# weiyithu/PV-RAFT

Hardware: NVIDIA H100
Metric: raft_sample_iters_per_sec (higher is better)
Workload: dtype f32

## Files before the change

pvraft_b200/csrc/tc_linear.cu:

```cuda
#include <cuda.h>
#include <stdlib.h>

#include "fixed_point.cuh"
#include "wgmma.cuh"

namespace pvraft {

constexpr int kTcThreads = 544;
constexpr int kTcEpiThreads = 256, kTcProducerWarp = 16;
constexpr int kTcM = 128, kTcKB = 32;
constexpr int kTcABytes = kTcM * kTcKB * 4;
constexpr int kTcMaxStages = 6;

#ifdef PVRAFT_TC_TIMELINE
__device__ unsigned long long g_tc_clock[64];
__device__ __forceinline__ unsigned long long gtimer() { unsigned long long t; asm volatile("mov.u64 %0, %%globaltimer;" : "=l"(t)); return t; }
#define TC_MARK(cond, slot) do { if (clk && (cond)) g_tc_clock[(slot)] = gtimer(); } while (0)
#else
#define TC_MARK(cond, slot) do { } while (0)
#endif

enum TcEpilogue { TC_EPI_PLAIN = 0, TC_EPI_GRU_ZR = 1, TC_EPI_GRU_Q = 2, TC_EPI_FLOW = 3 };

struct TcParams {
    const double* in_stats;
    const float* in_gamma;
    const float* in_beta;
    double in_count;
    int in_act;
    float in_slope;
    int minmax;
    int epi;
    const float* bias;
    const float* bias2;
    int out_act;
    const float* residual;
    float* out;
    float* out2;
    const float* h;
    const float* z;
    double* out_stats;
    int M, N, K, cout, pts_per_sample;
    const float* src[3];
    const float* src_min;
    int seg_kb[3];
    int stages;
    int w_resident;
    int settled;
    int dbg;
    int gn_kb;
    int out_ld;
    const float* tail;
// ... 259 lines not shown
                    const float4 aq = __ldg(reinterpret_cast<const float4*>(p.residual + (size_t)row * 64 + c + q * 4));
                    bq.x += aq.x; bq.y += aq.y; bq.z += aq.z; bq.w += aq.w;
                }
                o[q * 4 + 0] = tgru_blend(zv.x, hv.x, __uint_as_float(vq[q * 4 + 0]) + bq.x);
                o[q * 4 + 1] = tgru_blend(zv.y, hv.y, __uint_as_float(vq[q * 4 + 1]) + bq.y);
                o[q * 4 + 2] = tgru_blend(zv.z, hv.z, __uint_as_float(vq[q * 4 + 2]) + bq.z);
                o[q * 4 + 3] = tgru_blend(zv.w, hv.w, __uint_as_float(vq[q * 4 + 3]) + bq.w);
            }
            stage_store16(stg, lane, o, p.out + (size_t)(row0 + quad * 32) * 64 + c, 64);
        }
    }
}


struct TcCursor {
    int ti = 0, kb = 0, s = 0;
    unsigned phase = 0;
    __device__ __forceinline__ void next(int num_kb, int S) {
        if (++kb == num_kb) { kb = 0; ++ti; }
        if (++s == S) { s = 0; phase ^= 1u; }
    }
};

template <int N>
__device__ __forceinline__ void tc_mma_kblock(float (&acc)[64], unsigned long long a_hi, unsigned long long a_lo, unsigned long long b_hi,
                                              unsigned long long b_lo, int kb) {
#pragma unroll
    for (int k = 0; k < kTcKB / 8; ++k) {
        wgmma_tf32<N>(acc, wgmma_desc_k(a_hi, k), wgmma_desc_k(b_hi, k), (kb | k) != 0);
        wgmma_tf32<N>(acc, wgmma_desc_k(a_lo, k), wgmma_desc_k(b_hi, k), 1);
        wgmma_tf32<N>(acc, wgmma_desc_k(a_hi, k), wgmma_desc_k(b_lo, k), 1);
    }
}
__device__ __forceinline__ float4 tc_gn_act4(float4 x, const float4& sc, const float4& sh, const ActCoef& act) {
    x.x = apply_act(fmaf(x.x, sc.x, sh.x), act);
    x.y = apply_act(fmaf(x.y, sc.y, sh.y), act);
    x.z = apply_act(fmaf(x.z, sc.z, sh.z), act);
    x.w = apply_act(fmaf(x.w, sc.w, sh.w), act);
    return x;
}
__device__ __forceinline__ void tc_split_store(unsigned char* stage, int off, const float4& x) {
    float4 hi, lo;
    hi.x = tf32_rna(x.x); hi.y = tf32_rna(x.y); hi.z = tf32_rna(x.z); hi.w = tf32_rna(x.w);
    lo.x = tf32_rna(x.x - hi.x); lo.y = tf32_rna(x.y - hi.y); lo.z = tf32_rna(x.z - hi.z); lo.w = tf32_rna(x.w - hi.w);
    *reinterpret_cast<float4*>(stage + off) = hi;
    *reinterpret_cast<float4*>(stage + kTcABytes + off) = lo;
}
__host__ __device__ __forceinline__ int tc_acc_pitch(int n) { return ((n + 31) & ~31) + 4; }

template <int NT, bool DET>
__global__ void __launch_bounds__(kTcThreads, 1)
k_tc_linear(const __grid_constant__ CUtensorMap map_w_hi, const __grid_constant__ CUtensorMap map_w_lo,
            const __grid_constant__ CUtensorMap map_a0, const __grid_constant__ CUtensorMap map_a1,
            const __grid_constant__ CUtensorMap map_a2, const __grid_constant__ CUtensorMap map_min, const TcParams p) {
    extern __shared__ __align__(1024) unsigned char smem_raw[];
    unsigned char* tiles = smem_raw + ((1024u - ((unsigned)__cvta_generic_to_shared(smem_raw) & 1023u)) & 1023u);
    const int w_bytes = p.N * kTcKB * 4;
    const int w_off = 2 * kTcABytes;
    const int stage_bytes = w_off + (p.w_resident ? 0 : 2 * w_bytes);
    const int S = p.stages;
    const int num_kb = p.K / kTcKB;
    const int acc_pitch = tc_acc_pitch(NT);
    unsigned char* w_res = tiles + (size_t)S * stage_bytes;
    float* s_scale = reinterpret_cast<float*>(w_res + (p.w_resident ? (size_t)num_kb * 2 * w_bytes : 0));
    float* s_bias = s_scale + 4 * p.K;
    float* s_acc = s_bias + 2 * p.N;
    float* s_estage = s_acc + (size_t)kTcM * acc_pitch;
    float* s_part = s_estage + (p.epi == TC_EPI_GRU_ZR || p.epi == TC_EPI_GRU_Q ? 8 * 32 * kTcPitch16 : 0);
    __shared__ __align__(8) unsigned long long s_full[kTcMaxStages], s_empty[kTcMaxStages];
    __shared__ __align__(8) unsigned long long s_acc_full, s_acc_empty, s_w_full;
    const int warp = warp_id(), lane = lane_id();
    const int n_tiles = (p.M + kTcM - 1) / kTcM;
    const int my_tiles = blockIdx.x < n_tiles ? (n_tiles - 1 - blockIdx.x) / gridDim.x + 1 : 0;
    const int total_steps = my_tiles * num_kb;
#ifdef PVRAFT_TC_TIMELINE
    const bool clk = p.dbg && blockIdx.x == 0;
#endif
    TC_MARK(threadIdx.x == 0, 0);

    if (warp == kTcProducerWarp && lane == 0) {
// ... 131 lines not shown
          }
          wgmma_wait<0>();
          wgmma_fence_regs(acc);
          if (lane == 0) tmbar_arrive(&s_empty[prev_s]);
          prev_s = -1;
          TC_MARK(t == 0 && ti < 8, 16 + ti);
          tmbar_wait(&s_acc_empty, ((unsigned)ti & 1u) ^ 1u);
          float* a0 = s_acc + (size_t)(grp * 64 + (warp & 3) * 16 + (lane >> 2)) * acc_pitch + 2 * (lane & 3);
#pragma unroll
          for (int j = 0; j < NT / 8; ++j) {
              *reinterpret_cast<float2*>(a0 + 8 * j) = make_float2(acc[4 * j + 0], acc[4 * j + 1]);
              *reinterpret_cast<float2*>(a0 + (size_t)8 * acc_pitch + 8 * j) = make_float2(acc[4 * j + 2], acc[4 * j + 3]);
          }
          __syncwarp();
          if (lane == 0) tmbar_arrive(&s_acc_full);
        }
    } else {
        const int quad = warp & 3;
        const int half = warp >> 2;
        for (int ti = 0; ti < my_tiles; ++ti) {
            const int row0 = (blockIdx.x + ti * gridDim.x) * kTcM;
            tmbar_wait(&s_acc_full, (unsigned)ti & 1u);
            TC_MARK(threadIdx.x == 0 && ti < 4, 24 + ti);
            const int sample = row0 / p.pts_per_sample;
            tc_epilogue<DET>(p, s_acc, acc_pitch, quad, half, lane, row0, sample, s_bias, s_estage, s_part);
            __syncwarp();
            if (lane == 0) tmbar_arrive(&s_acc_empty);
            TC_MARK(threadIdx.x == 0 && ti < 4, 28 + ti);
        }
    }
    TC_MARK(threadIdx.x == 256, 1);
}

constexpr int kChThreads = 288;
constexpr int kChProducerWarp = 8;
constexpr int kChStages = 2;
constexpr int kChWBytes = 128 * kTcKB * 4;
constexpr int kChStageBytes = 2 * kTcABytes + 2 * kChWBytes;
constexpr int kChBufBytes = 2 * kTcABytes;
constexpr int kChSteps = 24;
enum ChSrc { CH_Y1 = 0, CH_KFEAT, CH_CFLOW, CH_NET, CH_INP, CH_X, CH_Y };

struct ChainParams {
    const double* y1_stats;
    const float *gn_gamma, *gn_beta;
    double gn_count;
    float gn_slope;
    const float *flow, *net;
    const float *b_cc, *b_m, *b_z, *b_r, *b_q;
    float *net_out, *p_out;
    int M, pts_per_sample;
};
struct ChainMaps {
    CUtensorMap a[5];
    CUtensorMap w_hi[5], w_lo[5];
};

__device__ __forceinline__ int ch_layer(int i) { return i < 6 ? 0 : i < 10 ? 1 : i < 16 ? 2 : i < 22 ? 3 : 4; }
__device__ __forceinline__ int ch_src(int i) {
    constexpr unsigned long long pairs = (unsigned long long)CH_X | (unsigned long long)CH_CFLOW << 4 | (unsigned long long)CH_NET << 8 |
                                         (unsigned long long)CH_INP << 12 | (unsigned long long)CH_Y << 16 | (unsigned long long)CH_X << 20 |
                                         (unsigned long long)CH_INP << 24 | (unsigned long long)CH_Y << 28 | (unsigned long long)CH_X << 32;
    return i < 4 ? CH_Y1 : i < 6 ? CH_KFEAT : (int)((pairs >> (4 * ((i - 6) >> 1))) & 15u);
}
__device__ __forceinline__ int ch_skb(int i) {
    return i < 4 ? i : (i < 6 ? i - 4 : (i - 6) & 1);
}
__device__ __forceinline__ int ch_first(int layer) { return layer == 0 ? 0 : layer == 1 ? 6 : layer == 2 ? 10 : layer == 3 ? 16 : 22; }
__device__ __forceinline__ int ch_w_bytes(int layer) { return (layer == 2 ? 128 : 64) * kTcKB * 4; }

__device__ __forceinline__ void ch_buf_store2(unsigned char* buf, int r, int c, float v0, float v1) {
    const int lc = (c & 31) >> 2;
    *reinterpret_cast<float2*>(buf + (c >> 5) * kTcABytes + r * 128 + ((lc ^ (r & 7)) << 4) + (c & 3) * 4) = make_float2(v0, v1);
}

template <int N>
__device__ __forceinline__ void ch_kblock(float (&acc)[64], int kb, int src, int skb, unsigned char* tiles, unsigned char* buf_x,
                                          unsigned char* buf_y, const float* g_scale, const float* g_shift, const ActCoef& iact,
                                          unsigned long long* s_full, unsigned long long* s_empty, TcCursor& cp, int grp, int t,
                                          int lane) {
    const int s = cp.s;
    tmbar_wait(&s_full[s], cp.phase);
    unsigned char* st = tiles + (size_t)s * kChStageBytes;
    const unsigned char* from = src == CH_X ? buf_x + skb * kTcABytes : src == CH_Y ? buf_y + skb * kTcABytes : st;
#pragma unroll
    for (int i = 0; i < 4; ++i) {
        const int c = t + i * 128, r = grp * 64 + (c >> 3), lc = c & 7;
        const int off = r * 128 + ((lc ^ (r & 7)) << 4);
        float4 x = *reinterpret_cast<const float4*>(from + off);
        if (src == CH_Y1) {
            const int k = skb * kTcKB + lc * 4;
            x = tc_gn_act4(x, *reinterpret_cast<const float4*>(g_scale + k), *reinterpret_cast<const float4*>(g_shift + k), iact);
        }
        tc_split_store(st, off, x);
    }
    asm volatile("fence.proxy.async.shared::cta;" ::: "memory");
    asm volatile("bar.sync %0, 128;" ::"r"(1 + grp) : "memory");
    const unsigned char* wb = st + 2 * kTcABytes;
    wgmma_fence_regs(acc);
    wgmma_fence();
    tc_mma_kblock<N>(acc, wgmma_desc(st + grp * 64 * 128), wgmma_desc(st + kTcABytes + grp * 64 * 128), wgmma_desc(wb),
                     wgmma_desc(wb + N * kTcKB * 4), kb);
    wgmma_commit();
    wgmma_wait<0>();
    if (lane == 0) tmbar_arrive(&s_empty[s]);
    cp.next(kChSteps, kChStages);
}
template <int N>
__device__ __forceinline__ void ch_layer_mma(float (&acc)[64], int i0, int nkb, unsigned char* tiles, unsigned char* buf_x,
                                             unsigned char* buf_y, const float* g_scale, const float* g_shift, const ActCoef& iact,
                                             unsigned long long* s_full, unsigned long long* s_empty, TcCursor& cp, int grp, int t,
                                             int lane) {
    for (int kb = 0; kb < nkb; ++kb)
        ch_kblock<N>(acc, kb, ch_src(i0 + kb), ch_skb(i0 + kb), tiles, buf_x, buf_y, g_scale, g_shift, iact, s_full, s_empty, cp, grp, t, lane);
    wgmma_fence_regs(acc);
}

__global__ void __launch_bounds__(kChThreads, 1)
k_update_chain(const __grid_constant__ ChainMaps maps, const ChainParams p) {
    extern __shared__ __align__(1024) unsigned char smem_raw[];
    unsigned char* tiles = smem_raw + ((1024u - ((unsigned)__cvta_generic_to_shared(smem_raw) & 1023u)) & 1023u);
    unsigned char* buf_x = tiles + (size_t)kChStages * kChStageBytes;
    unsigned char* buf_y = buf_x + kChBufBytes;
    float* s_scale = reinterpret_cast<float*>(buf_y + kChBufBytes);
    float* s_bias = s_scale + 2 * 256;
    __shared__ __align__(8) unsigned long long s_full[kChStages], s_empty[kChStages];
    const int warp = warp_id(), lane = lane_id();
    const int n_tiles = p.M / kTcM;
    const int my_tiles = blockIdx.x < n_tiles ? (n_tiles - 1 - blockIdx.x) / gridDim.x + 1 : 0;
    if (warp == kChProducerWarp && lane == 0) {
        for (int i = 0; i < 5; ++i) {
            asm volatile("prefetch.tensormap [%0];" ::"l"(&maps.a[i]) : "memory");
            asm volatile("prefetch.tensormap [%0];" ::"l"(&maps.w_hi[i]) : "memory");
            asm volatile("prefetch.tensormap [%0];" ::"l"(&maps.w_lo[i]) : "memory");
        }
        for (int s = 0; s < kChStages; ++s) { tmbar_init(&s_full[s], 1); tmbar_init(&s_empty[s], 8); }
        asm volatile("fence.mbarrier_init.release.cluster;" ::: "memory");
    }
    asm volatile("griddepcontrol.launch_dependents;" ::: "memory");
    __syncthreads();
    asm volatile("griddepcontrol.wait;" ::: "memory");
    if (threadIdx.x < 64) {
        const int c = threadIdx.x;
        s_bias[c] = __ldg(p.b_cc + c);
        s_bias[64 + c] = c < 61 ? __ldg(p.b_m + c) : 0.f;
        s_bias[128 + c] = __ldg(p.b_z + c);
        s_bias[192 + c] = __ldg(p.b_r + c);
        s_bias[256 + c] = __ldg(p.b_q + c);
    }
    __syncthreads();

    if (warp == kChProducerWarp) {
        if (lane == 0) {
            TcCursor cw;
            for (int step = 0; step < my_tiles * kChSteps; ++step, cw.next(kChSteps, kChStages)) {
                const int i = cw.kb, layer = ch_layer(i), src = ch_src(i);
                const int row0 = (blockIdx.x + cw.ti * gridDim.x) * kTcM;
                const int wb = ch_w_bytes(layer);
                const int lkb = i - ch_first(layer), skb = ch_skb(i);
                tmbar_wait(&s_empty[cw.s], cw.phase ^ 1u);
                unsigned char* st = tiles + (size_t)cw.s * kChStageBytes;
                tmbar_expect_tx(&s_full[cw.s], (unsigned)((src < CH_X ? kTcABytes : 0) + 2 * wb));
                if (src < CH_X) ttma_load_2d(st, &maps.a[src], &s_full[cw.s], skb * kTcKB, row0);
                ttma_load_2d(st + 2 * kTcABytes, &maps.w_hi[layer], &s_full[cw.s], lkb * kTcKB, 0);
                ttma_load_2d(st + 2 * kTcABytes + wb, &maps.w_lo[layer], &s_full[cw.s], lkb * kTcKB, 0);
            }
        }
        return;
    }

    const int grp = warp >> 2, t = threadIdx.x & 127;
    float* g_scale = s_scale + grp * 256;
    float* g_shift = g_scale + 128;
    const ActCoef iact = act_coef(PVRAFT_ACT_LRELU, p.gn_slope);
    const ActCoef relu = act_coef(PVRAFT_ACT_RELU, 0.f), none = act_coef(PVRAFT_ACT_NONE, 0.f);
    const int tiles_per_sample = p.pts_per_sample / kTcM;
    const int rq = (warp & 3) * 16 + (lane >> 2);
    const int cq = 2 * (lane & 3);
    int table_sample = -1;
    TcCursor cp;
    float acc[64], z[32];
    for (int ti = 0; ti < my_tiles; ++ti) {
        const int tile = blockIdx.x + ti * gridDim.x;
        const int row0 = tile * kTcM;
        const int sample = tile / tiles_per_sample;
        if (sample != table_sample) {
            table_sample = sample;
            asm volatile("bar.sync %0, 128;" ::"r"(1 + grp) : "memory");
            const double* sp = p.y1_stats + (size_t)sample * 16 + (t / 16) * 2;
            const double st[2] = {__ldcg(sp), __ldcg(sp + 1)};
            const GnAffine af = gn_affine(st, p.gn_count, __ldg(p.gn_gamma + t), __ldg(p.gn_beta + t));
            g_scale[t] = af.scale;
            g_shift[t] = af.shift;
            asm volatile("bar.sync %0, 128;" ::"r"(1 + grp) : "memory");
        }
        const int r_lo = grp * 64 + rq;
        ch_layer_mma<64>(acc, 0, 6, tiles, buf_x, buf_y, g_scale, g_shift, iact, s_full, s_empty, cp, grp, t, lane);
#pragma unroll
        for (int j = 0; j < 8; ++j)
#pragma unroll
            for (int h = 0; h < 2; ++h) {
                const int c = 8 * j + cq;
                ch_buf_store2(buf_x, r_lo + 8 * h, c, apply_act(acc[4 * j + 2 * h] + s_bias[c], relu), apply_act(acc[4 * j + 2 * h + 1] + s_bias[c + 1], relu));
            }
        asm volatile("bar.sync %0, 128;" ::"r"(1 + grp) : "memory");
        ch_layer_mma<64>(acc, 6, 4, tiles, buf_x, buf_y, g_scale, g_shift, iact, s_full, s_empty, cp, grp, t, lane);
#pragma unroll
        for (int j = 0; j < 8; ++j)
#pragma unroll
            for (int h = 0; h < 2; ++h) {
                const int c = 8 * j + cq, r = r_lo + 8 * h;
                float v0 = apply_act(acc[4 * j + 2 * h] + s_bias[64 + c], relu), v1 = apply_act(acc[4 * j + 2 * h + 1] + s_bias[64 + c + 1], relu);
                if (c >= 60) {
                    const float* fl = p.flow + (size_t)(row0 + r) * 3;
                    if (c == 62) { v0 = __ldcg(fl + 1); v1 = __ldcg(fl + 2); } else { v1 = __ldcg(fl); }
                }
                ch_buf_store2(buf_y, r, c, v0, v1);
            }
        asm volatile("bar.sync %0, 128;" ::"r"(1 + grp) : "memory");
        ch_layer_mma<128>(acc, 10, 6, tiles, buf_x, buf_y, g_scale, g_shift, iact, s_full, s_empty, cp, grp, t, lane);
#pragma unroll
        for (int j = 0; j < 8; ++j)
#pragma unroll
            for (int h = 0; h < 2; ++h) {
                const int c = 8 * j + cq, r = r_lo + 8 * h;
                const float2 hv = __ldcg(reinterpret_cast<const float2*>(p.net + (size_t)(row0 + r) * 64 + c));
                z[4 * j + 2 * h] = tsigmoid(acc[4 * j + 2 * h] + s_bias[128 + c]);
                z[4 * j + 2 * h + 1] = tsigmoid(acc[4 * j + 2 * h + 1] + s_bias[128 + c + 1]);
                ch_buf_store2(buf_x, r, c, tsigmoid(acc[32 + 4 * j + 2 * h] + s_bias[192 + c]) * hv.x,
                              tsigmoid(acc[32 + 4 * j + 2 * h + 1] + s_bias[192 + c + 1]) * hv.y);
            }
        asm volatile("bar.sync %0, 128;" ::"r"(1 + grp) : "memory");
        ch_layer_mma<64>(acc, 16, 6, tiles, buf_x, buf_y, g_scale, g_shift, iact, s_full, s_empty, cp, grp, t, lane);
#pragma unroll
        for (int j = 0; j < 8; ++j)
#pragma unroll
            for (int h = 0; h < 2; ++h) {
                const int c = 8 * j + cq, r = r_lo + 8 * h;
                const size_t g = (size_t)(row0 + r) * 64 + c;
                const float2 hv = __ldcg(reinterpret_cast<const float2*>(p.net + g));
                const float o0 = tgru_blend(z[4 * j + 2 * h], hv.x, acc[4 * j + 2 * h] + s_bias[256 + c]);
                const float o1 = tgru_blend(z[4 * j + 2 * h + 1], hv.y, acc[4 * j + 2 * h + 1] + s_bias[256 + c + 1]);
                *reinterpret_cast<float2*>(p.net_out + g) = make_float2(o0, o1);
                ch_buf_store2(buf_x, r, c, o0, o1);
            }
        asm volatile("bar.sync %0, 128;" ::"r"(1 + grp) : "memory");
        ch_layer_mma<64>(acc, 22, 2, tiles, buf_x, buf_y, g_scale, g_shift, iact, s_full, s_empty, cp, grp, t, lane);
#pragma unroll
        for (int j = 0; j < 8; ++j)
#pragma unroll
            for (int h = 0; h < 2; ++h) {
                const int c = 8 * j + cq, r = r_lo + 8 * h;
                *reinterpret_cast<float2*>(p.p_out + (size_t)(row0 + r) * 64 + c) =
                    make_float2(apply_act(acc[4 * j + 2 * h] + 0.f, none), apply_act(acc[4 * j + 2 * h + 1] + 0.f, none));
            }
    }
}

__global__ void k_weight_split(const float* __restrict__ w, int rows, int cols, int ld, int col0, int rows_pad, int cols_pad,
                               float* __restrict__ hi, float* __restrict__ lo) {
    const int i = blockIdx.x * blockDim.x + threadIdx.x;
    if (i >= rows_pad * cols_pad) return;
    const int r = i / cols_pad, c = i - r * cols_pad;
    float x = 0.f;
    if (r < rows && c < cols) x = __ldg(w + (size_t)r * ld + col0 + c);
    const float h = tf32_rna(x);
    hi[i] = h;
    lo[i] = tf32_rna(x - h);
}

typedef CUresult (*TcEncodeFn)(CUtensorMap*, CUtensorMapDataType, cuuint32_t, void*, const cuuint64_t*, const cuuint64_t*,
                               const cuuint32_t*, const cuuint32_t*, CUtensorMapInterleave, CUtensorMapSwizzle,
                               CUtensorMapL2promotion, CUtensorMapFloatOOBfill);
static TcEncodeFn tc_encode_fn() {
    static TcEncodeFn fn = nullptr;
    if (!fn) {
        void* p = nullptr;
        cudaDriverEntryPointQueryResult q;
        if (cudaGetDriverEntryPoint("cuTensorMapEncodeTiled", &p, cudaEnableDefault, &q) == cudaSuccess && q == cudaDriverEntryPointSuccess)
            fn = reinterpret_cast<TcEncodeFn>(p);
    }
    return fn;
}
static int tc_make_map(CUtensorMap* m, const float* base, long long rows, int cols, long long ld, int box_rows) {
    TcEncodeFn fn = tc_encode_fn();
    if (!fn) return fail(PVRAFT_ERR_UNSUPPORTED, "tc_linear: cuTensorMapEncodeTiled is not available from this driver");
    const cuuint64_t dims[2] = {(cuuint64_t)cols, (cuuint64_t)rows};
    const cuuint64_t strides[1] = {(cuuint64_t)ld * sizeof(float)};
    const cuuint32_t box[2] = {(cuuint32_t)kTcKB, (cuuint32_t)box_rows};
    const cuuint32_t estr[2] = {1, 1};
    const CUresult r = fn(m, CU_TENSOR_MAP_DATA_TYPE_FLOAT32, 2, const_cast<float*>(base), dims, strides, box, estr,
                          CU_TENSOR_MAP_INTERLEAVE_NONE, CU_TENSOR_MAP_SWIZZLE_128B, CU_TENSOR_MAP_L2_PROMOTION_L2_256B,
                          CU_TENSOR_MAP_FLOAT_OOB_FILL_NONE);
    if (r != CUDA_SUCCESS) return fail(PVRAFT_ERR_UNSUPPORTED, "tc_linear: cuTensorMapEncodeTiled failed (%d)", (int)r);
    return 0;
}

}

using namespace pvraft;

#ifdef PVRAFT_TC_TIMELINE
extern "C" __attribute__((visibility("default"))) int pvraft_tc_debug_clock(unsigned long long* host64) {
    return (int)cudaMemcpyFromSymbol(host64, g_tc_clock, sizeof(unsigned long long) * 64);
}
#endif

extern "C" int pvraft_tc_weight_split(const float* w, int rows, int cols, int ld, int col0, int rows_pad, int cols_pad, float* hi,
                                      float* lo, void* stream) {
    if (!w || !hi || !lo || rows <= 0 || cols <= 0 || rows_pad < rows || cols_pad < cols) return fail(PVRAFT_ERR_BAD_ARG, "tc_weight_split: bad argument");
    const int n = rows_pad * cols_pad;
    k_weight_split<<<(n + 255) / 256, 256, 0, (cudaStream_t)stream>>>(w, rows, cols, ld > 0 ? ld : cols, col0, rows_pad, cols_pad, hi, lo);
    return check_launch("tc_weight_split");
}

template <bool DET>
static int tc_linear_fwd(const pvraft_tc_linear_args* a, void* ws, void* stream) {
    if (!a || !a->in[0] || !a->w_hi || !a->w_lo || !a->out || (DET && a->out_stats && !ws)) return fail(PVRAFT_ERR_BAD_ARG, "tc_linear: null pointer");
    if (a->B <= 0 || a->N <= 0 || a->n_pad < 16 || a->n_pad > 128 || a->n_pad % 16) return fail(PVRAFT_ERR_BAD_ARG, "tc_linear: bad shape (n_pad=%d)", a->n_pad);
    if (a->N % kTcM) return fail(PVRAFT_ERR_UNSUPPORTED, "tc_linear: points per sample (%d) must be a multiple of 128", a->N);
    int K = 0;
    for (int s = 0; s < 3; ++s) {
        if (a->in[s] && (a->in_channels[s] <= 0 || a->in_channels[s] % kTcKB)) return fail(PVRAFT_ERR_UNSUPPORTED, "tc_linear: source %d has %d channels (multiple of 32 needed)", s, a->in_channels[s]);
        if (a->in[s]) K += a->in_channels[s];
    }
    if (K <= 0 || K > 512) return fail(PVRAFT_ERR_UNSUPPORTED, "tc_linear: K=%d", K);
    if (a->in_stats && (a->in_channels[0] % PVRAFT_GN_GROUPS || !a->in_gamma || !a->in_beta)) return fail(PVRAFT_ERR_BAD_ARG, "tc_linear: GroupNorm prologue needs gamma, beta and in_channels[0] %% 8 == 0");
    if (a->tail && (a->epilogue != TC_EPI_PLAIN || a->cout + 3 != a->n_pad || a->n_pad % 32 || a->residual || a->out_stats)) return fail(PVRAFT_ERR_BAD_ARG, "tc_linear: a tail needs the plain epilogue and cout + 3 == n_pad (multiple of 32)");
    if (a->in_min && !a->in_stats) return fail(PVRAFT_ERR_BAD_ARG, "tc_linear: in_min needs the GroupNorm prologue");
    if (a->out_stats && (a->epilogue != TC_EPI_PLAIN || a->cout % PVRAFT_GN_GROUPS || (a->cout / PVRAFT_GN_GROUPS) % 4)) return fail(PVRAFT_ERR_UNSUPPORTED, "tc_linear: out_stats needs a GroupNorm group size that is a multiple of 4 (cout=%d)", a->cout);
    if (a->epilogue < TC_EPI_PLAIN || a->epilogue > TC_EPI_FLOW) return fail(PVRAFT_ERR_BAD_ARG, "tc_linear: unknown epilogue %d", a->epilogue);
    if ((a->epilogue == TC_EPI_GRU_ZR || a->epilogue == TC_EPI_GRU_Q) && (a->cout != 64 || !a->h || (!a->bias && !a->residual))) return fail(PVRAFT_ERR_BAD_ARG, "tc_linear: GRU epilogues need cout=64, h and a bias or a pre-activation term");
    if (a->epilogue == TC_EPI_FLOW && (a->cout != 64 || a->n_pad != 64 || !a->bias || !a->w3 || !a->b3 || (a->coords2_out && !a->coords2) || (a->flow_out && (!a->coords2_out || !a->coords1)))) return fail(PVRAFT_ERR_BAD_ARG, "tc_linear: flow epilogue needs cout = n_pad = 64, bias, w3, b3 and consistent coordinate pointers");
    if (a->epilogue == TC_EPI_GRU_ZR && (a->n_pad != 128 || (!a->bias2 && !a->residual) || !a->out2)) return fail(PVRAFT_ERR_BAD_ARG, "tc_linear: GRU zr epilogue needs n_pad=128, bias2, out2");
    if (a->epilogue == TC_EPI_GRU_Q && (a->n_pad != 64 || !a->z)) return fail(PVRAFT_ERR_BAD_ARG, "tc_linear: GRU q epilogue needs n_pad=64 and z");
    const long long M = (long long)a->B * a->N;
    TcParams p{};
// ... 108 lines not shown
```

pvraft_b200/csrc/wgmma.cuh:

```cuda
#pragma once
#include "common.cuh"

namespace pvraft {

__device__ __forceinline__ unsigned long long wgmma_desc(const void* smem_tile) {
    unsigned long long d = 0;
    d |= (unsigned long long)((((unsigned)__cvta_generic_to_shared(smem_tile)) >> 4) & 0x3FFFu);
    d |= (unsigned long long)1 << 16;
    d |= (unsigned long long)64 << 32;
    d |= (unsigned long long)1 << 62;
    return d;
}
__device__ __forceinline__ unsigned long long wgmma_desc_k(unsigned long long d, int k) { return d + (unsigned long long)(k * 2); }

__device__ __forceinline__ void wgmma_fence() { asm volatile("wgmma.fence.sync.aligned;" ::: "memory"); }
__device__ __forceinline__ void wgmma_commit() { asm volatile("wgmma.commit_group.sync.aligned;" ::: "memory"); }
template <int N>
__device__ __forceinline__ void wgmma_wait() { asm volatile("wgmma.wait_group.sync.aligned %0;" ::"n"(N) : "memory"); }
__device__ __forceinline__ void wgmma_fence_regs(float (&d)[64]) {
#pragma unroll
    for (int i = 0; i < 64; ++i) asm volatile("" : "+f"(d[i])::"memory");
}

template <int N>
// ... 34 lines not shown
template <>
__device__ __forceinline__ void wgmma_tf32<80>(float (&d)[64], unsigned long long da, unsigned long long db, int accumulate) {
    asm volatile(
        "{\n\t.reg .pred p;\n\tsetp.ne.b32 p, %42, 0;\n\t"
        "wgmma.mma_async.sync.aligned.m64n80k8.f32.tf32.tf32 {%0, %1, %2, %3, %4, %5, %6, %7, %8, %9, %10, %11, %12, %13, %14, %15, %16, %17, %18, %19, %20, %21, %22, %23, %24, %25, %26, %27, %28, %29, %30, %31, %32, %33, %34, %35, %36, %37, %38, %39}, %40, %41, p, 1, 1;\n\t}"
        : "+f"(d[0]), "+f"(d[1]), "+f"(d[2]), "+f"(d[3]), "+f"(d[4]), "+f"(d[5]), "+f"(d[6]), "+f"(d[7]), "+f"(d[8]), "+f"(d[9]), "+f"(d[10]), "+f"(d[11]), "+f"(d[12]), "+f"(d[13]), "+f"(d[14]), "+f"(d[15]), "+f"(d[16]), "+f"(d[17]), "+f"(d[18]), "+f"(d[19]), "+f"(d[20]), "+f"(d[21]), "+f"(d[22]), "+f"(d[23]), "+f"(d[24]), "+f"(d[25]), "+f"(d[26]), "+f"(d[27]), "+f"(d[28]), "+f"(d[29]), "+f"(d[30]), "+f"(d[31]), "+f"(d[32]), "+f"(d[33]), "+f"(d[34]), "+f"(d[35]), "+f"(d[36]), "+f"(d[37]), "+f"(d[38]), "+f"(d[39])
        : "l"(da), "l"(db), "r"(accumulate));
}
template <>
__device__ __forceinline__ void wgmma_tf32<96>(float (&d)[64], unsigned long long da, unsigned long long db, int accumulate) {
    asm volatile(
        "{\n\t.reg .pred p;\n\tsetp.ne.b32 p, %50, 0;\n\t"
        "wgmma.mma_async.sync.aligned.m64n96k8.f32.tf32.tf32 {%0, %1, %2, %3, %4, %5, %6, %7, %8, %9, %10, %11, %12, %13, %14, %15, %16, %17, %18, %19, %20, %21, %22, %23, %24, %25, %26, %27, %28, %29, %30, %31, %32, %33, %34, %35, %36, %37, %38, %39, %40, %41, %42, %43, %44, %45, %46, %47}, %48, %49, p, 1, 1;\n\t}"
        : "+f"(d[0]), "+f"(d[1]), "+f"(d[2]), "+f"(d[3]), "+f"(d[4]), "+f"(d[5]), "+f"(d[6]), "+f"(d[7]), "+f"(d[8]), "+f"(d[9]), "+f"(d[10]), "+f"(d[11]), "+f"(d[12]), "+f"(d[13]), "+f"(d[14]), "+f"(d[15]), "+f"(d[16]), "+f"(d[17]), "+f"(d[18]), "+f"(d[19]), "+f"(d[20]), "+f"(d[21]), "+f"(d[22]), "+f"(d[23]), "+f"(d[24]), "+f"(d[25]), "+f"(d[26]), "+f"(d[27]), "+f"(d[28]), "+f"(d[29]), "+f"(d[30]), "+f"(d[31]), "+f"(d[32]), "+f"(d[33]), "+f"(d[34]), "+f"(d[35]), "+f"(d[36]), "+f"(d[37]), "+f"(d[38]), "+f"(d[39]), "+f"(d[40]), "+f"(d[41]), "+f"(d[42]), "+f"(d[43]), "+f"(d[44]), "+f"(d[45]), "+f"(d[46]), "+f"(d[47])
        : "l"(da), "l"(db), "r"(accumulate));
}
template <>
__device__ __forceinline__ void wgmma_tf32<112>(float (&d)[64], unsigned long long da, unsigned long long db, int accumulate) {
    asm volatile(
        "{\n\t.reg .pred p;\n\tsetp.ne.b32 p, %58, 0;\n\t"
        "wgmma.mma_async.sync.aligned.m64n112k8.f32.tf32.tf32 {%0, %1, %2, %3, %4, %5, %6, %7, %8, %9, %10, %11, %12, %13, %14, %15, %16, %17, %18, %19, %20, %21, %22, %23, %24, %25, %26, %27, %28, %29, %30, %31, %32, %33, %34, %35, %36, %37, %38, %39, %40, %41, %42, %43, %44, %45, %46, %47, %48, %49, %50, %51, %52, %53, %54, %55}, %56, %57, p, 1, 1;\n\t}"
        : "+f"(d[0]), "+f"(d[1]), "+f"(d[2]), "+f"(d[3]), "+f"(d[4]), "+f"(d[5]), "+f"(d[6]), "+f"(d[7]), "+f"(d[8]), "+f"(d[9]), "+f"(d[10]), "+f"(d[11]), "+f"(d[12]), "+f"(d[13]), "+f"(d[14]), "+f"(d[15]), "+f"(d[16]), "+f"(d[17]), "+f"(d[18]), "+f"(d[19]), "+f"(d[20]), "+f"(d[21]), "+f"(d[22]), "+f"(d[23]), "+f"(d[24]), "+f"(d[25]), "+f"(d[26]), "+f"(d[27]), "+f"(d[28]), "+f"(d[29]), "+f"(d[30]), "+f"(d[31]), "+f"(d[32]), "+f"(d[33]), "+f"(d[34]), "+f"(d[35]), "+f"(d[36]), "+f"(d[37]), "+f"(d[38]), "+f"(d[39]), "+f"(d[40]), "+f"(d[41]), "+f"(d[42]), "+f"(d[43]), "+f"(d[44]), "+f"(d[45]), "+f"(d[46]), "+f"(d[47]), "+f"(d[48]), "+f"(d[49]), "+f"(d[50]), "+f"(d[51]), "+f"(d[52]), "+f"(d[53]), "+f"(d[54]), "+f"(d[55])
        : "l"(da), "l"(db), "r"(accumulate));
}
template <>
__device__ __forceinline__ void wgmma_tf32<128>(float (&d)[64], unsigned long long da, unsigned long long db, int accumulate) {
    asm volatile(
        "{\n\t.reg .pred p;\n\tsetp.ne.b32 p, %66, 0;\n\t"
        "wgmma.mma_async.sync.aligned.m64n128k8.f32.tf32.tf32 {%0, %1, %2, %3, %4, %5, %6, %7, %8, %9, %10, %11, %12, %13, %14, %15, %16, %17, %18, %19, %20, %21, %22, %23, %24, %25, %26, %27, %28, %29, %30, %31, %32, %33, %34, %35, %36, %37, %38, %39, %40, %41, %42, %43, %44, %45, %46, %47, %48, %49, %50, %51, %52, %53, %54, %55, %56, %57, %58, %59, %60, %61, %62, %63}, %64, %65, p, 1, 1;\n\t}"
        : "+f"(d[0]), "+f"(d[1]), "+f"(d[2]), "+f"(d[3]), "+f"(d[4]), "+f"(d[5]), "+f"(d[6]), "+f"(d[7]), "+f"(d[8]), "+f"(d[9]), "+f"(d[10]), "+f"(d[11]), "+f"(d[12]), "+f"(d[13]), "+f"(d[14]), "+f"(d[15]), "+f"(d[16]), "+f"(d[17]), "+f"(d[18]), "+f"(d[19]), "+f"(d[20]), "+f"(d[21]), "+f"(d[22]), "+f"(d[23]), "+f"(d[24]), "+f"(d[25]), "+f"(d[26]), "+f"(d[27]), "+f"(d[28]), "+f"(d[29]), "+f"(d[30]), "+f"(d[31]), "+f"(d[32]), "+f"(d[33]), "+f"(d[34]), "+f"(d[35]), "+f"(d[36]), "+f"(d[37]), "+f"(d[38]), "+f"(d[39]), "+f"(d[40]), "+f"(d[41]), "+f"(d[42]), "+f"(d[43]), "+f"(d[44]), "+f"(d[45]), "+f"(d[46]), "+f"(d[47]), "+f"(d[48]), "+f"(d[49]), "+f"(d[50]), "+f"(d[51]), "+f"(d[52]), "+f"(d[53]), "+f"(d[54]), "+f"(d[55]), "+f"(d[56]), "+f"(d[57]), "+f"(d[58]), "+f"(d[59]), "+f"(d[60]), "+f"(d[61]), "+f"(d[62]), "+f"(d[63])
        : "l"(da), "l"(db), "r"(accumulate));
}

}
```

Before: 9312.

## Feed chain GEMM A operand from registers and overlap k-blocks with deeper pipeline

The fused GRU chain kernel now loads the A tile straight into wgmma register fragments and splits it into tf32 hi/lo parts in registers, instead of writing split tiles back to shared memory. That drops the shared-memory round trip, the proxy fence and the per-group named barrier, which become warp-level syncs. Two fragment buffers let one k-block's wgmma run while the next is prepared, using wait_group 1 with delayed stage release. Stages go from 2 to 3, and the thread count rises to 384 with setmaxnreg moving registers from producer warps to MMA warps. Risks are higher register pressure from the fragment arrays and correctness of the warp-only syncs on the shared buffers. Timing probes compiled under the timeline flag are also added.

```diff
diff --git a/pvraft_b200/csrc/tc_linear.cu b/pvraft_b200/csrc/tc_linear.cu
--- a/pvraft_b200/csrc/tc_linear.cu
+++ b/pvraft_b200/csrc/tc_linear.cu
@@ -16,8 +16,12 @@
 __device__ unsigned long long g_tc_clock[64];
 __device__ __forceinline__ unsigned long long gtimer() { unsigned long long t; asm volatile("mov.u64 %0, %%globaltimer;" : "=l"(t)); return t; }
 #define TC_MARK(cond, slot) do { if (clk && (cond)) g_tc_clock[(slot)] = gtimer(); } while (0)
+__device__ unsigned long long g_ch_clock[1024];
+constexpr int kChClkTile = 160;
+#define CH_MARK(cond, slot) do { if (blockIdx.x == 0 && (cond)) g_ch_clock[(slot)] = clock64(); } while (0)
 #else
 #define TC_MARK(cond, slot) do { } while (0)
+#define CH_MARK(cond, slot) do { } while (0)
 #endif
 
 enum TcEpilogue { TC_EPI_PLAIN = 0, TC_EPI_GRU_ZR = 1, TC_EPI_GRU_Q = 2, TC_EPI_FLOW = 3 };
@@ -343,20 +347,6 @@
         wgmma_tf32<N>(acc, wgmma_desc_k(a_hi, k), wgmma_desc_k(b_lo, k), 1);
     }
 }
-__device__ __forceinline__ float4 tc_gn_act4(float4 x, const float4& sc, const float4& sh, const ActCoef& act) {
-    x.x = apply_act(fmaf(x.x, sc.x, sh.x), act);
-    x.y = apply_act(fmaf(x.y, sc.y, sh.y), act);
-    x.z = apply_act(fmaf(x.z, sc.z, sh.z), act);
-    x.w = apply_act(fmaf(x.w, sc.w, sh.w), act);
-    return x;
-}
-__device__ __forceinline__ void tc_split_store(unsigned char* stage, int off, const float4& x) {
-    float4 hi, lo;
-    hi.x = tf32_rna(x.x); hi.y = tf32_rna(x.y); hi.z = tf32_rna(x.z); hi.w = tf32_rna(x.w);
-    lo.x = tf32_rna(x.x - hi.x); lo.y = tf32_rna(x.y - hi.y); lo.z = tf32_rna(x.z - hi.z); lo.w = tf32_rna(x.w - hi.w);
-    *reinterpret_cast<float4*>(stage + off) = hi;
-    *reinterpret_cast<float4*>(stage + kTcABytes + off) = lo;
-}
 __host__ __device__ __forceinline__ int tc_acc_pitch(int n) { return ((n + 31) & ~31) + 4; }
 
 template <int NT, bool DET>
@@ -554,11 +544,12 @@
     TC_MARK(threadIdx.x == 256, 1);
 }
 
-constexpr int kChThreads = 288;
+constexpr int kChThreads = 384;
 constexpr int kChProducerWarp = 8;
-constexpr int kChStages = 2;
+constexpr int kChProducerRegs = 40, kChMmaRegs = 232;
+constexpr int kChStages = 3;
 constexpr int kChWBytes = 128 * kTcKB * 4;
-constexpr int kChStageBytes = 2 * kTcABytes + 2 * kChWBytes;
+constexpr int kChStageBytes = kTcABytes + 2 * kChWBytes;
 constexpr int kChBufBytes = 2 * kTcABytes;
 constexpr int kChSteps = 24;
 enum ChSrc { CH_Y1 = 0, CH_KFEAT, CH_CFLOW, CH_NET, CH_INP, CH_X, CH_Y };
@@ -597,45 +588,84 @@
 }
 
 template <int N>
-__device__ __forceinline__ void ch_kblock(float (&acc)[64], int kb, int src, int skb, unsigned char* tiles, unsigned char* buf_x,
-                                          unsigned char* buf_y, const float* g_scale, const float* g_shift, const ActCoef& iact,
-                                          unsigned long long* s_full, unsigned long long* s_empty, TcCursor& cp, int grp, int t,
-                                          int lane) {
+__device__ __forceinline__ void ch_fence_acc(float (&d)[64]) {
+#pragma unroll
+    for (int i = 0; i < N / 2; ++i) asm volatile("" : "+f"(d[i])::"memory");
+}
+template <int N>
+__device__ __forceinline__ void ch_kblock(float (&acc)[64], unsigned (&fr)[4][2][4], int kb, int src, int skb, const unsigned char* tiles,
+                                          const unsigned char* buf_x, const unsigned char* buf_y, const float* g_scale,
+                                          const float* g_shift, const ActCoef& iact, unsigned long long* s_full,
+                                          unsigned long long* s_empty, TcCursor& cp, int& prev_s, int ra, int lane, bool mk) {
     const int s = cp.s;
     tmbar_wait(&s_full[s], cp.phase);
-    unsigned char* st = tiles + (size_t)s * kChStageBytes;
-    const unsigned char* from = src == CH_X ? buf_x + skb * kTcABytes : src == CH_Y ? buf_y + skb * kTcABytes : st;
-#pragma unroll
-    for (int i = 0; i < 4; ++i) {
-        const int c = t + i * 128, r = grp * 64 + (c >> 3), lc = c & 7;
-        const int off = r * 128 + ((lc ^ (r & 7)) << 4);
-        float4 x = *reinterpret_cast<const float4*>(from + off);
+    CH_MARK(mk && cp.ti < 4, 16 + cp.ti * kChClkTile + 4 * cp.kb + 0);
+    const unsigned char* st = tiles + (size_t)s * kChStageBytes;
+    const unsigned char* from = (src == CH_X ? buf_x + skb * kTcABytes : src == CH_Y ? buf_y + skb * kTcABytes : st) + ra * 128 + (lane & 3) * 4;
+    const int sw = lane >> 2;
+#pragma unroll
+    for (int k = 0; k < kTcKB / 8; ++k) {
+        float x[4];
+        x[0] = *reinterpret_cast<const float*>(from + (((2 * k) ^ sw) << 4));
+        x[1] = *reinterpret_cast<const float*>(from + 8 * 128 + (((2 * k) ^ sw) << 4));
+        x[2] = *reinterpret_cast<const float*>(from + (((2 * k + 1) ^ sw) << 4));
+        x[3] = *reinterpret_cast<const float*>(from + 8 * 128 + (((2 * k + 1) ^ sw) << 4));
         if (src == CH_Y1) {
-            const int k = skb * kTcKB + lc * 4;
-            x = tc_gn_act4(x, *reinterpret_cast<const float4*>(g_scale + k), *reinterpret_cast<const float4*>(g_shift + k), iact);
-        }
-        tc_split_store(st, off, x);
-    }
-    asm volatile("fence.proxy.async.shared::cta;" ::: "memory");
-    asm volatile("bar.sync %0, 128;" ::"r"(1 + grp) : "memory");
-    const unsigned char* wb = st + 2 * kTcABytes;
-    wgmma_fence_regs(acc);
+            const int c = skb * kTcKB + 8 * k + (lane & 3);
+            const float sc0 = g_scale[c], sh0 = g_shift[c], sc1 = g_scale[c + 4], sh1 = g_shift[c + 4];
+            x[0] = apply_act(fmaf(x[0], sc0, sh0), iact);
+            x[1] = apply_act(fmaf(x[1], sc0, sh0), iact);
+            x[2] = apply_act(fmaf(x[2], sc1, sh1), iact);
+            x[3] = apply_act(fmaf(x[3], sc1, sh1), iact);
+        }
+#pragma unroll
+        for (int j = 0; j < 4; ++j) {
+            const float hi = tf32_rna(x[j]);
+            fr[k][0][j] = __float_as_uint(hi);
+            fr[k][1][j] = __float_as_uint(tf32_rna(x[j] - hi));
+        }
+    }
+    CH_MARK(mk && cp.ti < 4, 16 + cp.ti * kChClkTile + 4 * cp.kb + 1);
+    const unsigned long long b_hi = wgmma_desc(st + kTcABytes), b_lo = wgmma_desc(st + kTcABytes + N * kTcKB * 4);
+    ch_fence_acc<N>(acc);
     wgmma_fence();
-    tc_mma_kblock<N>(acc, wgmma_desc(st + grp * 64 * 128), wgmma_desc(st + kTcABytes + grp * 64 * 128), wgmma_desc(wb),
-                     wgmma_desc(wb + N * kTcKB * 4), kb);
+#pragma unroll
+    for (int k = 0; k < kTcKB / 8; ++k) {
+        wgmma_tf32_ra<N>(acc, fr[k][0], wgmma_desc_k(b_hi, k), (kb | k) != 0);
+        wgmma_tf32_ra<N>(acc, fr[k][1], wgmma_desc_k(b_hi, k), 1);
+        wgmma_tf32_ra<N>(acc, fr[k][0], wgmma_desc_k(b_lo, k), 1);
+    }
     wgmma_commit();
+    CH_MARK(mk && cp.ti < 4, 16 + cp.ti * kChClkTile + 4 * cp.kb + 2);
+    wgmma_wait<1>();
+    if (kb > 0 && lane == 0) tmbar_arrive(&s_empty[prev_s]);
+    prev_s = s;
+    CH_MARK(mk && cp.ti < 4, 16 + cp.ti * kChClkTile + 4 * cp.kb + 3);
+    cp.next(kChSteps, kChStages);
+}
+template <int N, int I0, int NKB>
+__device__ __forceinline__ void ch_layer_mma(float (&acc)[64], unsigned (&fa)[4][2][4], unsigned (&fb)[4][2][4], const unsigned char* tiles,
+                                             const unsigned char* buf_x, const unsigned char* buf_y, const float* g_scale,
+                                             const float* g_shift, const ActCoef& iact, unsigned long long* s_full,
+                                             unsigned long long* s_empty, TcCursor& cp, int ra, int lane, bool mk) {
+    static_assert(NKB % 2 == 0, "k-blocks go in pairs, one per fragment buffer");
+    int prev_s = 0;
+#pragma unroll
+    for (int kb = 0; kb < NKB; kb += 2) {
+        ch_kblock<N>(acc, fa, kb, ch_src(I0 + kb), ch_skb(I0 + kb), tiles, buf_x, buf_y, g_scale, g_shift, iact, s_full, s_empty, cp, prev_s, ra, lane, mk);
+        ch_kblock<N>(acc, fb, kb + 1, ch_src(I0 + kb + 1), ch_skb(I0 + kb + 1), tiles, buf_x, buf_y, g_scale, g_shift, iact, s_full, s_empty, cp, prev_s, ra, lane, mk);
+    }
     wgmma_wait<0>();
-    if (lane == 0) tmbar_arrive(&s_empty[s]);
-    cp.next(kChSteps, kChStages);
-}
-template <int N>
-__device__ __forceinline__ void ch_layer_mma(float (&acc)[64], int i0, int nkb, unsigned char* tiles, unsigned char* buf_x,
-                                             unsigned char* buf_y, const float* g_scale, const float* g_shift, const ActCoef& iact,
-                                             unsigned long long* s_full, unsigned long long* s_empty, TcCursor& cp, int grp, int t,
-                                             int lane) {
-    for (int kb = 0; kb < nkb; ++kb)
-        ch_kblock<N>(acc, kb, ch_src(i0 + kb), ch_skb(i0 + kb), tiles, buf_x, buf_y, g_scale, g_shift, iact, s_full, s_empty, cp, grp, t, lane);
-    wgmma_fence_regs(acc);
+    ch_fence_acc<N>(acc);
+    if (lane == 0) tmbar_arrive(&s_empty[prev_s]);
+    __syncwarp();
+}
+
+__device__ __forceinline__ void ch_load_net(float2 (&hv)[16], const float* net, int r, int c) {
+#pragma unroll
+    for (int j = 0; j < 8; ++j)
+#pragma unroll
+        for (int h = 0; h < 2; ++h) hv[2 * j + h] = __ldcg(reinterpret_cast<const float2*>(net + (size_t)(r + 8 * h) * 64 + 8 * j + c));
 }
 
 __global__ void __launch_bounds__(kChThreads, 1)
@@ -650,6 +680,9 @@
     const int warp = warp_id(), lane = lane_id();
     const int n_tiles = p.M / kTcM;
     const int my_tiles = blockIdx.x < n_tiles ? (n_tiles - 1 - blockIdx.x) / gridDim.x + 1 : 0;
+#ifdef PVRAFT_TC_TIMELINE
+    if (blockIdx.x == 0 && threadIdx.x == 0) { g_ch_clock[0] = clock64(); g_ch_clock[1] = gtimer(); }
+#endif
     if (warp == kChProducerWarp && lane == 0) {
         for (int i = 0; i < 5; ++i) {
             asm volatile("prefetch.tensormap [%0];" ::"l"(&maps.a[i]) : "memory");
@@ -672,8 +705,9 @@
     }
     __syncthreads();
 
-    if (warp == kChProducerWarp) {
-        if (lane == 0) {
+    if (warp >= kChProducerWarp) {
+        asm volatile("setmaxnreg.dec.sync.aligned.u32 %0;" ::"n"(kChProducerRegs));
+        if (warp == kChProducerWarp && lane == 0) {
             TcCursor cw;
             for (int step = 0; step < my_tiles * kChSteps; ++step, cw.next(kChSteps, kChStages)) {
                 const int i = cw.kb, layer = ch_layer(i), src = ch_src(i);
@@ -684,13 +718,15 @@
                 unsigned char* st = tiles + (size_t)cw.s * kChStageBytes;
                 tmbar_expect_tx(&s_full[cw.s], (unsigned)((src < CH_X ? kTcABytes : 0) + 2 * wb));
                 if (src < CH_X) ttma_load_2d(st, &maps.a[src], &s_full[cw.s], skb * kTcKB, row0);
-                ttma_load_2d(st + 2 * kTcABytes, &maps.w_hi[layer], &s_full[cw.s], lkb * kTcKB, 0);
-                ttma_load_2d(st + 2 * kTcABytes + wb, &maps.w_lo[layer], &s_full[cw.s], lkb * kTcKB, 0);
+                ttma_load_2d(st + kTcABytes, &maps.w_hi[layer], &s_full[cw.s], lkb * kTcKB, 0);
+                ttma_load_2d(st + kTcABytes + wb, &maps.w_lo[layer], &s_full[cw.s], lkb * kTcKB, 0);
+                CH_MARK(cw.ti < 4, 16 + cw.ti * kChClkTile + 106 + i);
             }
         }
         return;
     }
 
+    asm volatile("setmaxnreg.inc.sync.aligned.u32 %0;" ::"n"(kChMmaRegs));
     const int grp = warp >> 2, t = threadIdx.x & 127;
     float* g_scale = s_scale + grp * 256;
     float* g_shift = g_scale + 128;
@@ -700,8 +736,11 @@
     const int rq = (warp & 3) * 16 + (lane >> 2);
     const int cq = 2 * (lane & 3);
     int table_sample = -1;
+    const int ra = grp * 64 + rq;
+    const bool mk = grp == 0 && t == 0;
     TcCursor cp;
     float acc[64], z[32];
+    unsigned fa[4][2][4], fb[4][2][4];
     for (int ti = 0; ti < my_tiles; ++ti) {
         const int tile = blockIdx.x + ti * gridDim.x;
         const int row0 = tile * kTcM;
@@ -716,22 +755,24 @@
             g_shift[t] = af.shift;
             asm volatile("bar.sync %0, 128;" ::"r"(1 + grp) : "memory");
         }
-        const int r_lo = grp * 64 + rq;
-        ch_layer_mma<64>(acc, 0, 6, tiles, buf_x, buf_y, g_scale, g_shift, iact, s_full, s_empty, cp, grp, t, lane);
+        ch_layer_mma<64, 0, 6>(acc, fa, fb, tiles, buf_x, buf_y, g_scale, g_shift, iact, s_full, s_empty, cp, ra, lane, mk);
+        CH_MARK(mk && ti < 4, 16 + ti * kChClkTile + 96 + 0);
 #pragma unroll
         for (int j = 0; j < 8; ++j)
 #pragma unroll
             for (int h = 0; h < 2; ++h) {
                 const int c = 8 * j + cq;
-                ch_buf_store2(buf_x, r_lo + 8 * h, c, apply_act(acc[4 * j + 2 * h] + s_bias[c], relu), apply_act(acc[4 * j + 2 * h + 1] + s_bias[c + 1], relu));
-            }
-        asm volatile("bar.sync %0, 128;" ::"r"(1 + grp) : "memory");
-        ch_layer_mma<64>(acc, 6, 4, tiles, buf_x, buf_y, g_scale, g_shift, iact, s_full, s_empty, cp, grp, t, lane);
+                ch_buf_store2(buf_x, ra + 8 * h, c, apply_act(acc[4 * j + 2 * h] + s_bias[c], relu), apply_act(acc[4 * j + 2 * h + 1] + s_bias[c + 1], relu));
+            }
+        __syncwarp();
+        CH_MARK(mk && ti < 4, 16 + ti * kChClkTile + 96 + 1);
+        ch_layer_mma<64, 6, 4>(acc, fa, fb, tiles, buf_x, buf_y, g_scale, g_shift, iact, s_full, s_empty, cp, ra, lane, mk);
+        CH_MARK(mk && ti < 4, 16 + ti * kChClkTile + 96 + 2);
 #pragma unroll
         for (int j = 0; j < 8; ++j)
 #pragma unroll
             for (int h = 0; h < 2; ++h) {
-                const int c = 8 * j + cq, r = r_lo + 8 * h;
+                const int c = 8 * j + cq, r = ra + 8 * h;
                 float v0 = apply_act(acc[4 * j + 2 * h] + s_bias[64 + c], relu), v1 = apply_act(acc[4 * j + 2 * h + 1] + s_bias[64 + c + 1], relu);
                 if (c >= 60) {
                     const float* fl = p.flow + (size_t)(row0 + r) * 3;
@@ -739,44 +780,55 @@
                 }
                 ch_buf_store2(buf_y, r, c, v0, v1);
             }
-        asm volatile("bar.sync %0, 128;" ::"r"(1 + grp) : "memory");
-        ch_layer_mma<128>(acc, 10, 6, tiles, buf_x, buf_y, g_scale, g_shift, iact, s_full, s_empty, cp, grp, t, lane);
+        __syncwarp();
+        CH_MARK(mk && ti < 4, 16 + ti * kChClkTile + 96 + 3);
+        ch_layer_mma<128, 10, 6>(acc, fa, fb, tiles, buf_x, buf_y, g_scale, g_shift, iact, s_full, s_empty, cp, ra, lane, mk);
+        CH_MARK(mk && ti < 4, 16 + ti * kChClkTile + 96 + 4);
+        float2 hv[16];
+        ch_load_net(hv, p.net, row0 + ra, cq);
 #pragma unroll
         for (int j = 0; j < 8; ++j)
 #pragma unroll
             for (int h = 0; h < 2; ++h) {
-                const int c = 8 * j + cq, r = r_lo + 8 * h;
-                const float2 hv = __ldcg(reinterpret_cast<const float2*>(p.net + (size_t)(row0 + r) * 64 + c));
+                const int c = 8 * j + cq, r = ra + 8 * h;
                 z[4 * j + 2 * h] = tsigmoid(acc[4 * j + 2 * h] + s_bias[128 + c]);
                 z[4 * j + 2 * h + 1] = tsigmoid(acc[4 * j + 2 * h + 1] + s_bias[128 + c + 1]);
-                ch_buf_store2(buf_x, r, c, tsigmoid(acc[32 + 4 * j + 2 * h] + s_bias[192 + c]) * hv.x,
-                              tsigmoid(acc[32 + 4 * j + 2 * h + 1] + s_bias[192 + c + 1]) * hv.y);
-            }
-        asm volatile("bar.sync %0, 128;" ::"r"(1 + grp) : "memory");
-        ch_layer_mma<64>(acc, 16, 6, tiles, buf_x, buf_y, g_scale, g_shift, iact, s_full, s_empty, cp, grp, t, lane);
+                ch_buf_store2(buf_x, r, c, tsigmoid(acc[32 + 4 * j + 2 * h] + s_bias[192 + c]) * hv[2 * j + h].x,
+                              tsigmoid(acc[32 + 4 * j + 2 * h + 1] + s_bias[192 + c + 1]) * hv[2 * j + h].y);
+            }
+        __syncwarp();
+        CH_MARK(mk && ti < 4, 16 + ti * kChClkTile + 96 + 5);
+        ch_layer_mma<64, 16, 6>(acc, fa, fb, tiles, buf_x, buf_y, g_scale, g_shift, iact, s_full, s_empty, cp, ra, lane, mk);
+        CH_MARK(mk && ti < 4, 16 + ti * kChClkTile + 96 + 6);
+        ch_load_net(hv, p.net, row0 + ra, cq);
 #pragma unroll
         for (int j = 0; j < 8; ++j)
 #pragma unroll
             for (int h = 0; h < 2; ++h) {
-                const int c = 8 * j + cq, r = r_lo + 8 * h;
+                const int c = 8 * j + cq, r = ra + 8 * h;
                 const size_t g = (size_t)(row0 + r) * 64 + c;
-                const float2 hv = __ldcg(reinterpret_cast<const float2*>(p.net + g));
-                const float o0 = tgru_blend(z[4 * j + 2 * h], hv.x, acc[4 * j + 2 * h] + s_bias[256 + c]);
-                const float o1 = tgru_blend(z[4 * j + 2 * h + 1], hv.y, acc[4 * j + 2 * h + 1] + s_bias[256 + c + 1]);
+                const float o0 = tgru_blend(z[4 * j + 2 * h], hv[2 * j + h].x, acc[4 * j + 2 * h] + s_bias[256 + c]);
+                const float o1 = tgru_blend(z[4 * j + 2 * h + 1], hv[2 * j + h].y, acc[4 * j + 2 * h + 1] + s_bias[256 + c + 1]);
                 *reinterpret_cast<float2*>(p.net_out + g) = make_float2(o0, o1);
                 ch_buf_store2(buf_x, r, c, o0, o1);
             }
-        asm volatile("bar.sync %0, 128;" ::"r"(1 + grp) : "memory");
-        ch_layer_mma<64>(acc, 22, 2, tiles, buf_x, buf_y, g_scale, g_shift, iact, s_full, s_empty, cp, grp, t, lane);
+        __syncwarp();
+        CH_MARK(mk && ti < 4, 16 + ti * kChClkTile + 96 + 7);
+        ch_layer_mma<64, 22, 2>(acc, fa, fb, tiles, buf_x, buf_y, g_scale, g_shift, iact, s_full, s_empty, cp, ra, lane, mk);
+        CH_MARK(mk && ti < 4, 16 + ti * kChClkTile + 96 + 8);
 #pragma unroll
         for (int j = 0; j < 8; ++j)
 #pragma unroll
             for (int h = 0; h < 2; ++h) {
-                const int c = 8 * j + cq, r = r_lo + 8 * h;
+                const int c = 8 * j + cq, r = ra + 8 * h;
                 *reinterpret_cast<float2*>(p.p_out + (size_t)(row0 + r) * 64 + c) =
                     make_float2(apply_act(acc[4 * j + 2 * h] + 0.f, none), apply_act(acc[4 * j + 2 * h + 1] + 0.f, none));
             }
-    }
+        CH_MARK(mk && ti < 4, 16 + ti * kChClkTile + 96 + 9);
+    }
+#ifdef PVRAFT_TC_TIMELINE
+    if (blockIdx.x == 0 && threadIdx.x == 0) { g_ch_clock[2] = clock64(); g_ch_clock[3] = gtimer(); }
+#endif
 }
 
 __global__ void k_weight_split(const float* __restrict__ w, int rows, int cols, int ld, int col0, int rows_pad, int cols_pad,
@@ -825,6 +877,9 @@
 #ifdef PVRAFT_TC_TIMELINE
 extern "C" __attribute__((visibility("default"))) int pvraft_tc_debug_clock(unsigned long long* host64) {
     return (int)cudaMemcpyFromSymbol(host64, g_tc_clock, sizeof(unsigned long long) * 64);
+}
+extern "C" __attribute__((visibility("default"))) int pvraft_chain_debug_clock(unsigned long long* host1024) {
+    return (int)cudaMemcpyFromSymbol(host1024, g_ch_clock, sizeof(unsigned long long) * 1024);
 }
 #endif
 
diff --git a/pvraft_b200/csrc/wgmma.cuh b/pvraft_b200/csrc/wgmma.cuh
--- a/pvraft_b200/csrc/wgmma.cuh
+++ b/pvraft_b200/csrc/wgmma.cuh
@@ -90,4 +90,24 @@
         : "l"(da), "l"(db), "r"(accumulate));
 }
 
+template <int N>
+__device__ __forceinline__ void wgmma_tf32_ra(float (&d)[64], const unsigned (&a)[4], unsigned long long db, int accumulate);
+
+template <>
+__device__ __forceinline__ void wgmma_tf32_ra<64>(float (&d)[64], const unsigned (&a)[4], unsigned long long db, int accumulate) {
+    asm volatile(
+        "{\n\t.reg .pred p;\n\tsetp.ne.b32 p, %37, 0;\n\t"
+        "wgmma.mma_async.sync.aligned.m64n64k8.f32.tf32.tf32 {%0, %1, %2, %3, %4, %5, %6, %7, %8, %9, %10, %11, %12, %13, %14, %15, %16, %17, %18, %19, %20, %21, %22, %23, %24, %25, %26, %27, %28, %29, %30, %31}, {%32, %33, %34, %35}, %36, p, 1, 1;\n\t}"
+        : "+f"(d[0]), "+f"(d[1]), "+f"(d[2]), "+f"(d[3]), "+f"(d[4]), "+f"(d[5]), "+f"(d[6]), "+f"(d[7]), "+f"(d[8]), "+f"(d[9]), "+f"(d[10]), "+f"(d[11]), "+f"(d[12]), "+f"(d[13]), "+f"(d[14]), "+f"(d[15]), "+f"(d[16]), "+f"(d[17]), "+f"(d[18]), "+f"(d[19]), "+f"(d[20]), "+f"(d[21]), "+f"(d[22]), "+f"(d[23]), "+f"(d[24]), "+f"(d[25]), "+f"(d[26]), "+f"(d[27]), "+f"(d[28]), "+f"(d[29]), "+f"(d[30]), "+f"(d[31])
+        : "r"(a[0]), "r"(a[1]), "r"(a[2]), "r"(a[3]), "l"(db), "r"(accumulate));
 }
+template <>
+__device__ __forceinline__ void wgmma_tf32_ra<128>(float (&d)[64], const unsigned (&a)[4], unsigned long long db, int accumulate) {
+    asm volatile(
+        "{\n\t.reg .pred p;\n\tsetp.ne.b32 p, %69, 0;\n\t"
+        "wgmma.mma_async.sync.aligned.m64n128k8.f32.tf32.tf32 {%0, %1, %2, %3, %4, %5, %6, %7, %8, %9, %10, %11, %12, %13, %14, %15, %16, %17, %18, %19, %20, %21, %22, %23, %24, %25, %26, %27, %28, %29, %30, %31, %32, %33, %34, %35, %36, %37, %38, %39, %40, %41, %42, %43, %44, %45, %46, %47, %48, %49, %50, %51, %52, %53, %54, %55, %56, %57, %58, %59, %60, %61, %62, %63}, {%64, %65, %66, %67}, %68, p, 1, 1;\n\t}"
+        : "+f"(d[0]), "+f"(d[1]), "+f"(d[2]), "+f"(d[3]), "+f"(d[4]), "+f"(d[5]), "+f"(d[6]), "+f"(d[7]), "+f"(d[8]), "+f"(d[9]), "+f"(d[10]), "+f"(d[11]), "+f"(d[12]), "+f"(d[13]), "+f"(d[14]), "+f"(d[15]), "+f"(d[16]), "+f"(d[17]), "+f"(d[18]), "+f"(d[19]), "+f"(d[20]), "+f"(d[21]), "+f"(d[22]), "+f"(d[23]), "+f"(d[24]), "+f"(d[25]), "+f"(d[26]), "+f"(d[27]), "+f"(d[28]), "+f"(d[29]), "+f"(d[30]), "+f"(d[31]), "+f"(d[32]), "+f"(d[33]), "+f"(d[34]), "+f"(d[35]), "+f"(d[36]), "+f"(d[37]), "+f"(d[38]), "+f"(d[39]), "+f"(d[40]), "+f"(d[41]), "+f"(d[42]), "+f"(d[43]), "+f"(d[44]), "+f"(d[45]), "+f"(d[46]), "+f"(d[47]), "+f"(d[48]), "+f"(d[49]), "+f"(d[50]), "+f"(d[51]), "+f"(d[52]), "+f"(d[53]), "+f"(d[54]), "+f"(d[55]), "+f"(d[56]), "+f"(d[57]), "+f"(d[58]), "+f"(d[59]), "+f"(d[60]), "+f"(d[61]), "+f"(d[62]), "+f"(d[63])
+        : "r"(a[0]), "r"(a[1]), "r"(a[2]), "r"(a[3]), "l"(db), "r"(accumulate));
+}
+
+}
```

Result: faster. 9581 (median of 6 runs) (+2.9%).
